# Mictronics/pluto-gps-sim

Measured on AMD Instinct MI355X. Metric: IQ samples/sec (whole node) at 16 channels; bit-exact int16 IQ vs CPU ref, higher is better.
Workload: dtype f64 NCOs (exact), i32 accumulate of packed int16 I/Q

## Files before the change

pluto-gps-sim_amd/csrc/gpsbb.hip:

```cpp
#include <hip/hip_runtime.h>

#include <algorithm>
#include <cctype>
#include <cmath>
#include <cstdio>
#include <cstdlib>
#include <cstring>
#include <new>
#include <condition_variable>
#include <functional>
#include <mutex>
#include <thread>
#include <chrono>
#include <vector>

#include "gpsbb.h"
#include "gpsbb_kernels.hip.h"
#include "gpsbb_noise.hip.h"
#include "gpsbb_interf.hip.h"
#include "gpsbb_level.hip.h"
#include "gpsbb_events.hip.h"
#include "gpsbb_dense.hip.h"
#include "gpsbb_despread.hip.h"
#include "gpsbb_despread_lags.hip.h"
// ... 3941 lines not shown
    HIPCHK(h, hipGetLastError());
    HIPCHK(h, hipStreamSynchronize(h->s_compute));
    HIPCHK(h, hipMemcpy(maxima, d_mx, mx_bytes, hipMemcpyDeviceToHost));
    HIPCHK(h, hipMemcpy(counts, d_cnt, cnt_bytes, hipMemcpyDeviceToHost));
    (void)hipFree(d_mx);
    (void)hipFree(d_cnt);
    if (which)
        *which = pl.ev_all_dense ? 2 : 1;
    return GPSBB_OK;
}

extern "C" int gpsbb_test_state_log2(gpsbb_batch_t *b)
{
    return b ? b->plan.st_log2 : GPSBB_E_BADARG;
}

static unsigned long long fnv1a(const void *p, size_t n)
{
    unsigned long long h = 0xcbf29ce484222325ull;
    for (size_t i = 0; i < n; i++)
        h = (h ^ ((const uint8_t *)p)[i]) * 0x100000001b3ull;
    return h;
}

template <class T>
static unsigned long long fnv1a(const std::vector<T> &v, bool defined = true)
{
    return defined ? fnv1a(v.data(), v.size() * sizeof(T)) : 0ull;
}

// ... 33 lines not shown
extern "C" int gpsbb_test_table_digest(gpsbb_batch_t *b, unsigned long long out[3])
{
    if (!b || !out || !b->ran || !b->plan.ev)
        return GPSBB_E_STATE;
    gpsbb *h = b->h;
    const BatchPlan &pl = b->plan;
    const int rc = gpsbb_sync(h);
    if (rc != GPSBB_OK)
        return rc;
    const BatchDev p = batch_dev(b, b->sets[b->last_set]);
    auto mix = [](unsigned long long z) { z ^= z >> 31; z *= 0xBF58476D1CE4E5B9ull; z ^= z >> 29; return z; };
    const size_t nst = (size_t)pl.nstates;
    const size_t nx = (size_t)pl.nblocks * 2 * pl.nch * nst, nn = (size_t)pl.nblocks * pl.nch * nst, ne = (size_t)pl.nblocks * pl.nch;
    const int dg = pl.ev_dense || (pl.flags & GPSBB_FIXED_CARRIER) ? 0 : (int)GPSBB_KNOB_LONG("GPSBB_EV_STATE_LOG2", GPSBB_EV_STATE_LOG2);
    const int tstep = 1 << (dg > pl.st_log2 ? dg : pl.st_log2);
    std::vector<unsigned long long> hx(nx);
    std::vector<uint32_t> hn(nn);
    std::vector<gpsbb_chan_state_t> he(ne);
    HIPCHK(h, hipMemcpy(hx.data(), p.tile_x, nx * 8, hipMemcpyDeviceToHost));
    HIPCHK(h, hipMemcpy(hn.data(), p.tile_nav, nn * 4, hipMemcpyDeviceToHost));
    HIPCHK(h, hipMemcpy(he.data(), p.end, ne * sizeof(gpsbb_chan_state_t), hipMemcpyDeviceToHost));
    out[0] = out[1] = out[2] = 0;
    std::vector<gpsbb_chan_t> hc(ne);
    HIPCHK(h, hipMemcpy(hc.data(), p.ch, ne * sizeof(gpsbb_chan_t), hipMemcpyDeviceToHost));
    for (size_t k = 0; k < ne; k++) {
        if (hc[k].prn <= 0)
            continue;
        const size_t blk = k / (size_t)pl.nch, i = k % (size_t)pl.nch;
        for (int kind = 0; kind < 2; kind++)
            for (int t = 0; t < pl.ntiles; t += tstep) {
                const size_t at = (blk * 2 * pl.nch + 2 * i + kind) * (size_t)pl.ntiles + t;
                out[0] += mix(hx[(blk * 2 * pl.nch + 2 * i + kind) * nst + (t >> pl.st_log2)] + 0x9E3779B97F4A7C15ull * (at + 1));
            }
        for (int t = 0; t < pl.ntiles; t += tstep) {
            const size_t at = k * (size_t)pl.ntiles + t;
            out[1] += mix((unsigned long long)(hn[k * nst + (t >> pl.st_log2)] & 3u) + 0x9E3779B97F4A7C15ull * (at + 1));
        }
        unsigned long long w[5];
        memcpy(w, &he[k], sizeof w);
        for (int q = 0; q < 4; q++)
            out[2] += mix(w[q] + 0x9E3779B97F4A7C15ull * (k * 5 + q + 1));
        out[2] += mix((unsigned long long)(uint32_t)he[k].codeCA + 0x9E3779B97F4A7C15ull * (k * 5 + 5));
    }
    return GPSBB_OK;
}

extern "C" void gpsbb_test_budgets(double out[3])
// ... 79 lines not shown
```

pluto-gps-sim_amd/csrc/gpsbb_despread.hip.h:

```cpp
#ifndef GPSBB_DESPREAD_HIP_H
#define GPSBB_DESPREAD_HIP_H

#include "gpsbb_dense.hip.h"
#include "gpsbb_noise.hip.h"
#include "gpsbb_interf.hip.h"

namespace gpsbb_impl {

constexpr int DS_WG = 256;
constexpr int DS_WAVES = DS_WG / 64;
constexpr int DS_CHUNK = 4;
constexpr int DS_SC16 = 0;

struct DsArgs {
    const uint32_t *iq;
    unsigned long long *out;
    unsigned long long *n_exact;
    int32_t *ctr;
    int seg_tiles, nseg, chunk, wgs_per_block;
    int shift8;
    uint32_t danger;
    NoiseArgs nz;
    const int2 *ntab;
    InterfArgs it;
};

typedef short ds_s16x2 __attribute__((ext_vector_type(2)));

struct DsLds {
    uint2 rep[2][512];
    uint32_t chips[GPSBB_MAX_CHAN][32];
};

__device__ __forceinline__ uint32_t ds_pair(int lo, int hi) { return ((uint32_t)lo & 0xffffu) | ((uint32_t)hi << 16); }

__device__ __noinline__ uint32_t ds_exact_sample(double xt, double yt, double S, double sc, uint32_t down, uint32_t nav, int n,
                                                 const uint32_t *chips)
{
    int64_t wraps = 0;
    const double x = code_jump(xt, sc, (int64_t)n, &wraps);
    const uint32_t neg = wraps > 0 ? (nav >> 1) & 1u : nav & 1u;
    const double cp = carr_jump(yt * (1.0 / 512.0), (down ? -S : S) * (1.0 / 512.0), (int64_t)n);
    const int it = (int)(cp * 512.0) & 511;
    const int ci = (int)x;
    const uint32_t bit = (chips[(ci >> 5) & 31] >> (ci & 31)) & 1u;
    return (uint32_t)it | (((bit ^ 1u) ^ neg) << 9);
}

__device__ __forceinline__ uint32_t ds_model_sample(double nn, double S, double sc, double yg, double xg, uint32_t flip, uint32_t nav,
                                                    const uint32_t *chips, uint32_t danger, bool &bad)
{
    const double y = __fma_rn(nn, S, yg), x = __fma_rn(nn, sc, xg);
    bad = min((uint32_t)__double2loint(y), (uint32_t)__double2loint(x)) < danger;
    const uint32_t it = ((uint32_t)__double2hiint(y) & 511u) ^ flip;
    uint32_t c = (uint32_t)__double2hiint(x) & 0xfffffu;
    const bool rolled = c >= (uint32_t)GPSBB_CA_LEN;
    c -= rolled ? (uint32_t)GPSBB_CA_LEN : 0u;
    const uint32_t bit = (chips[(c >> 5) & 31u] >> (c & 31u)) & 1u;
    const uint32_t neg = rolled ? (nav >> 1) & 1u : nav & 1u;
    return it | (((bit ^ 1u) ^ neg) << 9);
}

struct DsRepTab {
    const uint2 *rep;
    __device__ __forceinline__ void operator()(uint32_t idx, int *c, int *s) const
    {
        const uint32_t v = rep[idx].x;
// ... 98 lines not shown
            const int seg = wt / a.seg_tiles;
            if (seg != run_seg) {
                flush();
                run_seg = seg;
            }
            const int left = p.nsamp - wt * TILE - lane;
            uint32_t u[SPT];
#pragma unroll
            for (int j = 0; j < SPT; j++)
                u[j] = j * 64 < left ? iqb[(size_t)wt * TILE + j * 64 + lane] : 0u;
#pragma unroll
            for (int j = 0; j < SPT; j++)
                u[j] = j * 64 < left ? ds_view<VIEW, NOISE, INTERF>(u[j], (unsigned long long)b * (unsigned long long)p.nsamp +
                                                                              (unsigned long long)(wt * TILE + j * 64 + lane), a, ntab, L.rep[0])
                                     : 0u;
            const int g = wt >> SG;
            const double n0 = (double)((wt & ((1 << SG) - 1)) * TILE + lane);
            for (uint32_t mk = act_mask; mk; mk &= mk - 1) {
                const int i = __builtin_ctz(mk);
                const double S = scalar_load(&kb[i].S), sc = scalar_load(&kb[i].sc);
                const uint32_t down = scalar_load(&kb[i].down) != 0 ? 1u : 0u;
                const double xt = txb[(size_t)(2 * i) * nst + g], yt = txb[(size_t)(2 * i + 1) * nst + g];
                const uint32_t nav = tnb[(size_t)i * nst + g];
                const double yg = (down ? 512.0 - yt : yt) + guard, xg = xt + guard;
                const uint32_t flip = down ? 511u : 0u;
                const uint32_t *chips = L.chips[i];
                int pi = 0, pq = 0;
                uint32_t bad = 0u;
#pragma unroll
                for (int j = 0; j < SPT; j++) {
                    bool bj;
                    const uint32_t r = ds_model_sample(n0 + (double)(j * 64), S, sc, yg, xg, flip, nav, chips, a.danger, bj);
                    bad |= bj ? 1u << j : 0u;
                    const uint2 t = (&L.rep[0][0])[r];
                    pi = __builtin_amdgcn_sdot2(__builtin_bit_cast(ds_s16x2, u[j]), __builtin_bit_cast(ds_s16x2, t.x), pi, false);
                    pq = __builtin_amdgcn_sdot2(__builtin_bit_cast(ds_s16x2, u[j]), __builtin_bit_cast(ds_s16x2, t.y), pq, false);
                }
                if (__builtin_expect(__builtin_amdgcn_ballot_w64(bad != 0u) != 0ull, 0)) {
#pragma unroll 1
                    for (int j = 0; j < SPT; j++) {
                        if (!((bad >> j) & 1u) || j * 64 >= left)
                            continue;
                        uint32_t uw = 0u;
#pragma unroll
                        for (int q = 0; q < SPT; q++)
                            uw = q == j ? u[q] : uw;
                        bool bj;
                        const uint32_t rm = ds_model_sample(n0 + (double)(j * 64), S, sc, yg, xg, flip, nav, chips, a.danger, bj);
                        const uint32_t re = ds_exact_sample(xt, yt, S, sc, down, nav, (wt & ((1 << SG) - 1)) * TILE + j * 64 + lane, chips);
                        const uint2 tm = (&L.rep[0][0])[rm], te = (&L.rep[0][0])[re];
                        const ds_s16x2 uj = __builtin_bit_cast(ds_s16x2, uw);
                        pi += __builtin_amdgcn_sdot2(uj, __builtin_bit_cast(ds_s16x2, te.x), 0, false) -
                              __builtin_amdgcn_sdot2(uj, __builtin_bit_cast(ds_s16x2, tm.x), 0, false);
                        pq += __builtin_amdgcn_sdot2(uj, __builtin_bit_cast(ds_s16x2, te.y), 0, false) -
                              __builtin_amdgcn_sdot2(uj, __builtin_bit_cast(ds_s16x2, tm.y), 0, false);
                        n_exact++;
                    }
                }
                long long si = pi, sq = pq;
#pragma unroll
                for (int off = 32; off > 0; off >>= 1) {
                    si += __shfl_xor(si, off);
                    sq += __shfl_xor(sq, off);
                }
// ... 18 lines not shown
```

pluto-gps-sim_amd/csrc/gpsbb_despread_lags.hip.h:

```cpp
#ifndef GPSBB_DESPREAD_LAGS_HIP_H
#define GPSBB_DESPREAD_LAGS_HIP_H

#include "gpsbb_despread.hip.h"

namespace gpsbb_impl {

constexpr int DSL_MAX_LAGS = GPSBB_DESPREAD_MAX_LAGS;
constexpr int DSL_HALO = GPSBB_DESPREAD_MAX_LAG;
constexpr int DSL_STRIP = TILE + 2 * DSL_HALO;
constexpr int DSL_RED_ROW = 64 + 4;
static_assert(DSL_HALO == 64 && 2 * DSL_MAX_LAGS == 16 && GPSBB_MAX_CHAN == 16,
              "one halo group per side; lane (v, q) = (2 * lag + component, channel & 3), register set channel >> 2");

struct DslArgs {
    DsArgs d;
    int lags[DSL_MAX_LAGS];
    int nlags;
    int halo_lo, halo_hi;
};

template <int VIEW, bool NOISE, int SG, bool INTERF = false>
__global__ __launch_bounds__(DS_WG) void k_despread_lags(BatchDev p, DslArgs al)
{
    __shared__ DsLds L;
// ... 71 lines not shown
            __builtin_amdgcn_wave_barrier();
            const int m0 = wt * TILE - DSL_HALO + lane;
#pragma unroll 2
            for (int g = 0; g < SPT + 2; g++) {
                const int m = m0 + g * 64;
                const bool need = (g != 0 || al.halo_lo) && (g != SPT + 1 || al.halo_hi);
                uint32_t w = 0u;
                if (need && m >= 0 && m < p.nsamp)
                    w = ds_view<VIEW, NOISE, INTERF>(iqb[m], (unsigned long long)b * (unsigned long long)p.nsamp + (unsigned long long)m, a,
                                                     ntab, L.rep[0]);
                vw[g * 64 + lane] = w;
            }
            __builtin_amdgcn_fence(__ATOMIC_ACQ_REL, "workgroup");
            __builtin_amdgcn_wave_barrier();
            const int left = p.nsamp - wt * TILE - lane;
            const int g = wt >> SG;
            const int ns = (wt & ((1 << SG) - 1)) * TILE + lane;
            const double n0 = (double)ns;
            for (uint32_t mk = act_mask; mk; mk &= mk - 1) {
                const int i = __builtin_ctz(mk);
                const double S = scalar_load(&kb[i].S), sc = scalar_load(&kb[i].sc);
                const uint32_t down = scalar_load(&kb[i].down) != 0 ? 1u : 0u;
                const double xt = txb[(size_t)(2 * i) * nst + g], yt = txb[(size_t)(2 * i + 1) * nst + g];
                const uint32_t nav = tnb[(size_t)i * nst + g];
                const double yg = (down ? 512.0 - yt : yt) + guard, xg = xt + guard;
                const uint32_t flip = down ? 511u : 0u;
                const uint32_t *chips = L.chips[i];
                uint2 t[SPT];
                uint32_t bad = 0u;
#pragma unroll
                for (int j = 0; j < SPT; j++) {
                    bool bj;
                    const uint32_t r = ds_model_sample(n0 + (double)(j * 64), S, sc, yg, xg, flip, nav, chips, a.danger, bj);
                    const bool is = j * 64 < left;
                    bad |= bj && is ? 1u << j : 0u;
                    const uint2 tj = (&L.rep[0][0])[r];
                    t[j] = is ? tj : make_uint2(0u, 0u);
                }
                if (__builtin_expect(__builtin_amdgcn_ballot_w64(bad != 0u) != 0ull, 0)) {
#pragma unroll 1
                    for (int j = 0; j < SPT; j++) {
                        if (!((bad >> j) & 1u))
                            continue;
                        const uint32_t re = ds_exact_sample(xt, yt, S, sc, down, nav, ns + j * 64, chips);
                        const uint2 te = (&L.rep[0][0])[re];
#pragma unroll
                        for (int q = 0; q < SPT; q++)
                            t[q] = q == j ? te : t[q];
                        n_exact++;
                    }
                }
                __builtin_amdgcn_fence(__ATOMIC_ACQ_REL, "workgroup");
                __builtin_amdgcn_wave_barrier();
#pragma unroll 1
                for (int l = 0; l < nlags; l++) {
                    const int lag = __builtin_amdgcn_readfirstlane(lagv[l]);
                    const uint32_t *__restrict__ wl = vw + (DSL_HALO + lane + lag);
                    uint32_t w[SPT];
#pragma unroll
// ... 43 lines not shown
```

pluto-gps-sim_amd/csrc/gpsbb_events.hip.h:

```cpp
#ifndef GPSBB_EVENTS_HIP_H
#define GPSBB_EVENTS_HIP_H

#include <cstddef>
#include <type_traits>

#include "gpsbb_kernels.hip.h"

namespace gpsbb_impl {

#ifndef GPSBB_EV_WG
#define GPSBB_EV_WG 1024
#endif
constexpr int EV_WG = GPSBB_EV_WG;
constexpr int EV_WAVES = EV_WG / 64;
constexpr int EV_KC_MAX = 4;
constexpr int EV_AMP_PAD = EV_KC_MAX;
constexpr int EV_AMP_STRIDE = 512 + EV_AMP_PAD + 4;
constexpr int EV_CHIP_LEN = 1024 + 544;
constexpr int EV_KC_DENSE = EV_KC_MAX + 1;
#ifndef GPSBB_EV_CHUNK
#define GPSBB_EV_CHUNK 4
#endif
constexpr int EV_CHUNK = GPSBB_EV_CHUNK;
constexpr int PD_CHUNK = 2;
// ... 4 lines not shown
#define GPSBB_EV_MODEL_ERR_OWN 1
#endif
#ifndef EV_T_EPS
#define EV_T_EPS 0x1p-29
#endif
#define EV_GUARD 0x1p+20

#ifndef GPSBB_EV_STATE_LOG2
#define GPSBB_EV_STATE_LOG2 1
#endif
constexpr int EV_STATE_LOG2_MAX = 2;
static_assert(GPSBB_EV_STATE_LOG2 >= 0 && GPSBB_EV_STATE_LOG2 <= EV_STATE_LOG2_MAX, "state granule: 1, 2 or 4 tiles");
constexpr bool ev_granule_fits(int g) { return ((double)(TILE << g) + (double)(SPT - 1)) * 0x1p-44 + 1.5 * 0x1p-32 <= EV_MODEL_ERR; }
#ifdef GPSBB_EV_MODEL_ERR_OWN
static_assert(ev_granule_fits(EV_STATE_LOG2_MAX), "the model of the largest state granule must stay inside the error budget");
#endif

#define GPSBB_EV_SETTLE_CLAIM() asm volatile("s_waitcnt vmcnt(0)" ::: "memory")

constexpr int EV_CHIP_LEN_SHORT = 1104;
constexpr int EV_AMP_STRIDE_LONG = 512 + 272 + EV_AMP_PAD;
template <int AMP_STRIDE, int CHIP_LEN>
struct EvLdsT {
    static constexpr int AMP = AMP_STRIDE, CHIPS = CHIP_LEN;
    static constexpr bool UNMASKED = AMP_STRIDE >= EV_AMP_STRIDE_LONG;
    uint32_t amp[GPSBB_MAX_CHAN][AMP_STRIDE];
    uint32_t D[EV_WAVES][16][64];
    double tstate[EV_WAVES][2][2 * GPSBB_MAX_CHAN];
    double tstep[2 * GPSBB_MAX_CHAN];
    uint16_t chip2[GPSBB_MAX_CHAN][CHIP_LEN];
// ... 32 lines not shown
                 "ds_add_u32 %0, %3 offset:%4"
                 : "+v"(drow)
                 : "s"(wave << 4), "v"(pos_hi), "v"(v), "n"(offsetof(LDS, D))
                 );
}

__device__ __forceinline__ uint32_t signed_by(uint32_t x, uint32_t m) { return (x ^ m) - m; }

template <class T>
__device__ __forceinline__ T scalar_load(const T *p)
{
    typedef const __attribute__((address_space(4))) T *cptr_t;
    return *(cptr_t)(uintptr_t)p;
}

template <bool FIXED, class LDS>
__device__ __forceinline__ uint32_t ev_exact_run_body(LDS &L, int wave, int lane, int i, const EvConst *kbi, const double *tile_x,
                                                      int ntiles, uint32_t nb, int n_off, uint32_t fx_phase, int32_t fx_step)
{
    constexpr bool fixed = FIXED;
    const bool down = kbi->down != 0;
    const double S = down ? -kbi->S : kbi->S, sc = kbi->sc;
    const double xt = tile_x[(size_t)(2 * i) * ntiles], yt = tile_x[(size_t)(2 * i + 1) * ntiles];
    int64_t wraps = 0;
    double x = code_jump(xt, sc, (int64_t)n_off, &wraps);
    uint32_t dbm = (wraps > 0 ? (nb >> 1) & 1u : nb & 1u) ? 0xffffffffu : 0u;
    const uint32_t dbm_next = ((nb >> 1) & 1u) ? 0xffffffffu : 0u;
    const double s = S * (1.0 / 512.0);
    double cp = carr_jump(yt * (1.0 / 512.0), s, (int64_t)n_off);
    uint32_t prev = 0, first = 0;
    uint32_t ph = fx_phase + (uint32_t)n_off * (uint32_t)fx_step;
#pragma unroll 1
    for (int j = 0; j < SPT; j++) {
        const int it = fixed ? (int)((ph >> 16) & 0x1ffu)
                             : ((int)(cp * 512.0) & 511);
        const int ci = (int)x;
        const uint32_t m = (uint32_t)(int32_t)(int8_t)(L.chip2[i][ci] & 0xffu) ^ dbm;
        const uint32_t v = signed_by(L.amp[i][down ? 511 - it : it], m);
        if (j == 0)
            first = v;
        else
            __hip_atomic_fetch_add(&L.D[wave][j - 1][lane], v - prev, __ATOMIC_RELAXED, __HIP_MEMORY_SCOPE_WORKGROUP);
        prev = v;
        if (code_step(x, sc))
// ... 2 lines not shown
        ph += (uint32_t)fx_step;
    }
    return first;
}

struct EvFixed {
    const uint32_t *ph;
    const int32_t *st;
    int n0;
};

template <class LDS>
__device__ __noinline__ uint32_t ev_exact_run(LDS &L, int wave, int lane, int i, const EvConst *kbi, const double *tile_x,
                                              int ntiles, uint32_t nb, int n_off)
{
    return ev_exact_run_body<false>(L, wave, lane, i, kbi, tile_x, ntiles, nb, n_off, 0u, 0);
}
template <class LDS>
__device__ __noinline__ uint32_t ev_exact_run_fixed(LDS &L, int wave, int lane, int i, const EvConst *kbi, const double *tile_x,
                                                    int ntiles, uint32_t nb, int n_off, uint32_t fx_phase, int32_t fx_step)
{
    return ev_exact_run_body<true>(L, wave, lane, i, kbi, tile_x, ntiles, nb, n_off, fx_phase, fx_step);
}

struct EvK {
    double S, rS, sc, rsc;
    uint32_t danger;
    uint32_t chip_base;
    uint32_t amp_base;
};
constexpr uint32_t EV_GUARD_HI = 0x41300000u;
template <class LDS>
__device__ __forceinline__ EvK ev_load_k(const LDS &L, const EvConst *kb, int i)
{
    EvK k;
    typedef uint32_t u32x8 __attribute__((ext_vector_type(8)));
    typedef uint32_t u32x4 __attribute__((ext_vector_type(4)));
// ... 88 lines not shown
    EvExactAt a;
    if (!T.sg) {
        a.tile_x = T.tile_x;
        a.stride = T.ntiles;
        a.nb = ((T.dbits >> i) & 1u) | (((T.dnext >> i) & 1u) << 1);
        a.n_skip = 0;
    } else {
        const int nst = (T.ntiles + (1 << T.sg) - 1) >> T.sg, g = T.wt >> T.sg;
        a.tile_x = T.tile_x + g;
        a.stride = nst;
        a.nb = ((T.dbits >> i) & 1u) | (((T.dnext >> i) & 1u) << 1);
        a.n_skip = (T.wt & ((1 << T.sg) - 1)) * TILE;
    }
    return a;
}

template <int KC, bool DF, bool FIXED, class LDS>
__device__ __forceinline__ void ev_second(LDS &L, uint32_t &drow, int wave, int lane, int i, EvHalf<KC> &h, uint32_t db, uint32_t db_next,
                                          unsigned long long live_mask, const EvConst *kb, const EvTile &T,
                                          double off, uint32_t &acc0, unsigned long long *n_exact, const EvFixed &fx)
{
    const uint32_t ma = (uint32_t)(int32_t)(int8_t)(h.ch2 & 0xffu), mb = (uint32_t)(int32_t)(int8_t)(h.ch2 >> 8);
    uint32_t m0, m1;
    if (DF) {
        m0 = ma ^ (h.c0 >= 1023 ? db_next : db);
        m1 = mb ^ (h.c0 >= 1022 ? db_next : db);
    } else {
        m0 = ma ^ db;
        m1 = mb ^ db;
    }
    uint32_t hc = m0 == m1 ? EV_SAT_HI : h.hc;

    if (__builtin_expect(h.um != 0ull, 0)) {
        const unsigned long long um = h.um & live_mask;
        GPSBB_EV_SETTLE_CLAIM();
        if ((um >> lane) & 1ull) {
#pragma unroll
            for (int k = 0; k < KC; k++)
                h.hk[k] = EV_SAT_HI;
            hc = EV_SAT_HI;
            h.A[0] = 0;
            const EvExactAt x = ev_exact_at(T, i);
            if (FIXED)
                acc0 += ev_exact_run_fixed(L, wave, lane, i, kb + i, x.tile_x, x.stride, x.nb, x.n_skip + (int)off,
                                           fx.ph[i] + (uint32_t)fx.n0 * (uint32_t)fx.st[i], fx.st[i]);
            else
                acc0 += ev_exact_run(L, wave, lane, i, kb + i, x.tile_x, x.stride, x.nb, x.n_skip + (int)off);
            atomicAdd(n_exact, 1ull);
        }
    }

    {
        const uint32_t c = acc0 - m0;
        asm("v_xad_u32 %0, %1, %2, %3" : "=v"(acc0) : "v"(h.A[0]), "v"(m0), "v"(c));
    }
    uint32_t Ax = h.A[KC];
#pragma unroll
    for (int k = KC - 1; k >= 0; k--) {
        const bool before = h.hk[k] < hc;
        const uint32_t mk = before ? m0 : m1;
// ... 229 lines not shown
    const int ntw = p.ntiles;
    const int nch2 = 2 * p.nch;
    uint32_t mk[EV_KC_MAX];
    uint32_t mkd;
    {
        const bool act = lane < p.nch && cb[lane < p.nch ? lane : 0].prn > 0;
        const int kc = act ? kb[lane].kc : 0;
#pragma unroll
        for (int k = 0; k < EV_KC_MAX; k++)
            mk[k] = (uint32_t)__ballot(act && (kc == k + 1 || (k == 0 && kc < 1)));
        mkd = DENSE ? (uint32_t)__ballot(act && kc == EV_KC_DENSE) : 0u;
    }
    const bool chain_lane = lane < nch2;
    const bool mirror = chain_lane && (lane & 1) && kb[lane >> 1].down != 0;
    constexpr int sg = SG;
    const int nst = SG ? p.nstates : ntw;
    const double *__restrict__ txb = p.tile_x + (size_t)b * nst * nch2;
    const uint32_t *__restrict__ tnb = p.tile_nav + (size_t)b * p.nch * nst;
    const double off = (double)(lane * SPT);
    const double guard_w = EV_GUARD + ((chain_lane && !(FIXED && (lane & 1))) ? kb[lane >> 1].W : 0.0);
    const double mirror_at = FIXED ? 512.0 - 0x1p-16 : 512.0;
    unsigned long long *n_exact = p.hazards + 2;
    const uint32_t dwave = lds_addr_of(&L.D[wave][0][0]);
    const uint32_t d_col = dwave + (uint32_t)lane * 4u;
    const uint32_t t_wr = (dwave + (uint32_t)lane * 64u) ^ ((((uint32_t)lane >> 1) & 3u) << 4);
    const uint32_t t_rd = dwave + ((uint32_t)lane >> 2) * 64u + ((((uint32_t)lane & 3u) ^ (((uint32_t)lane >> 3) & 3u)) << 4);
    const uint32_t t_zero = dwave + (uint32_t)lane * 16u;
    uint32_t drow = (uint32_t)lane * 4u;

    int base = 0;
// ... 1 lines not shown
        base = atomicAdd(&p.tile_ctr[b], p.ev_chunk);
    base = __builtin_amdgcn_readfirstlane(base);
    int pos = 0;
    int pending = 0;
    unsigned tiles_rendered = 0;
    double ts_v = 0.0;
    uint32_t nav_v = 0;
    const auto stage_tile = [&](int t, uint32_t &dbits, uint32_t &dnext) {
        const int r = t & ((1 << sg) - 1);
        bool rolled_over = false;
        uint32_t ln = (uint32_t)lane;
        asm volatile("" : "+v"(ln));
        if (chain_lane) {
            double v = (mirror ? mirror_at - ts_v : ts_v) + guard_w;
            if (sg) {
                if (r)
                    v = __fma_rn(SG == 1 ? (double)TILE : (double)(r * TILE), L.tstep[ln], v);
                const uint32_t ip = (uint32_t)__double2hiint(v) - EV_GUARD_HI;
                const uint32_t red = (ln & 1u) ? (ip & ~511u) : (ip >= (uint32_t)GPSBB_CA_LEN + 1u ? (uint32_t)GPSBB_CA_LEN : 0u);
                v -= (double)red;
                rolled_over = !(ln & 1u) && red != 0u;
            }
            L.tstate[wave][0][ln] = v;
        }
        dbits = (uint32_t)__ballot(nav_v & 1u);
        dnext = (uint32_t)__ballot(nav_v & 2u);
        if (sg && r) {
            uint32_t ro = (uint32_t)__ballot(rolled_over) & 0x55555555u;
            ro = (ro | (ro >> 1)) & 0x33333333u;
            ro = (ro | (ro >> 2)) & 0x0f0f0f0fu;
            ro = (ro | (ro >> 4)) & 0x00ff00ffu;
            ro = (ro | (ro >> 8)) & 0x0000ffffu;
            dbits = (dbits & ~ro) | (dnext & ro);
        }
    };
    uint32_t t_dbits = 0u, t_dnext = 0u;
    const auto fetch_granule = [&](int g) {
        uint32_t ln = (uint32_t)lane;
        asm volatile("" : "+v"(ln));
        const uint32_t at = ln * (uint32_t)nst + (uint32_t)g;
        if (chain_lane)
            ts_v = txb[at];
        if (lane < p.nch)
            nav_v = tnb[at];
    };
    if (base < ntw) {
        fetch_granule(base >> sg);
        stage_tile(base, t_dbits, t_dnext);
    }
    while (base < ntw) {
        const int wt = base + pos;
        const int r = wt & ((1 << sg) - 1);
        EvTile T;
        T.ts = L.tstate[wave][0];
        T.tile_x = sg ? txb : txb + wt;
        T.ntiles = ntw;
        T.wt = wt;
// ... 153 lines not shown
```

pluto-gps-sim_amd/csrc/gpsbb_laps.hip.h:

```cpp
#ifndef GPSBB_LAPS_HIP_H
#define GPSBB_LAPS_HIP_H

#include "gpsbb_walk.hip.h"

namespace gpsbb_impl {

#ifdef GPSBB_LAP_WAVES
#define GPSBB_LAP_OCC __attribute__((amdgpu_waves_per_eu(GPSBB_LAP_WAVES, GPSBB_LAP_WAVES)))
#else
#define GPSBB_LAP_OCC
#endif
constexpr int LAP_WG = 256;
constexpr uint32_t LAPF_ACTIVE = 1u;
constexpr uint32_t LAPF_HEAD = 2u;
constexpr uint32_t LAPF_CONT = 4u;
constexpr uint32_t LAPF_CONST = 8u;
constexpr uint32_t LAPF_BAD = 16u;
constexpr uint32_t ST_LAP_PLAN = 8u;

struct LapBC {
    double phi;
    double s;
    double R1;
    double Rphi;
// ... 310 lines not shown
template <int KIND>
__device__ __forceinline__ void lap_enter_block(const BatchDev &p, const LapDev &L, int i, LapLane<KIND> &w)
{
    const LapBC bc = L.bc[((size_t)KIND * p.nch + i) * (size_t)p.nblocks + w.b];
    w.s = bc.s;
    w.bcflags = bc.flags;
    w.c0 = bc.c0;
    const uint64_t sb = f64_bits(bc.s);
    w.es = (int)((sb >> 52) & 0x7ff);
    w.tiemask = (sb << 1) == 0ull ? 0ull : walk_tiemask(sb);
    w.neg = bc.s < 0.0;
    w.tt = ((w.tiemask >> (((KIND == NCO_CARR ? 1022 : 1023 + 9) - w.es) & 63)) & 1ull) != 0ull;
    w.nmax = (w.b == w.bt) ? w.nt : p.nsamp;
}

template <int KIND, int SG = -1>
__device__ __forceinline__ void lap_nav_out(const BatchDev &p, int i, LapLane<KIND> &w, bool on, int n_excl, uint32_t bits)
{
    const uint32_t tsl = (uint32_t)__builtin_ctz(TILE) + (uint32_t)(SG >= 0 ? SG : p.st_log2);
    const int TS = 1 << tsl;
    typedef uint32_t lap_u4 __attribute__((ext_vector_type(4)));
    const int t = w.navt;
    int t_end = (int)(((uint32_t)n_excl + (uint32_t)(TS - 1)) >> tsl);
    t_end = t_end < p.nstates ? t_end : p.nstates;
    int cnt = on && t_end > t ? t_end - t : 0;
    if (cnt > 0)
        w.navt = t_end;
    if (!__ballot(cnt > 0))
        return;
    uint32_t *pn = p.tile_nav + ((size_t)w.b * (size_t)p.nch + i) * (size_t)p.nstates + t;
// ... 8 lines not shown
            }
        }
        if (quad)
            *reinterpret_cast<lap_u4 *>(pn) = b4;
        if (cnt > 0 && !oct && !quad)
            *pn = bits;
        const int adv = oct ? 8 : (quad ? 4 : (cnt > 0 ? 1 : 0));
        pn += adv;
        cnt -= adv;
    }
}

template <int KIND, bool WIDE, int SG = -1>
__device__ __forceinline__ void lap_emit_row(const BatchDev &p, int i, bool on, int b, int n, int k, double x, double S, uint32_t bits)
{
    const uint32_t tsl = (uint32_t)__builtin_ctz(TILE) + (uint32_t)(SG >= 0 ? SG : p.st_log2);
    const int TS = 1 << tsl;
    int t = (int)(((uint32_t)n + (uint32_t)(TS - 1)) >> tsl);
    int t_end = (int)((uint32_t)(n + k) >> tsl) + 1;
    t_end = t_end < p.nstates ? t_end : p.nstates;
    int cnt = on ? t_end - t : 0;
    cnt = cnt < 0 ? 0 : cnt;
    if (!__ballot(cnt > 0))
        return;
    double *__restrict__ tx = p.tile_x + ((size_t)b * (2 * (size_t)p.nch) + 2 * i + KIND) * (size_t)p.nstates;
    unsigned long long big = __ballot(cnt > 24);
    if (big && __popcll(big) <= 6) {
        const int lane = (int)__lane_id();
        while (big) {
            const int src = __builtin_ctzll(big);
            big &= big - 1;
            const int t0 = __builtin_amdgcn_readlane(t, src), c = __builtin_amdgcn_readlane(cnt, src);
            const int nn = __builtin_amdgcn_readlane(n, src);
            const double xx = bits_f64(readlane_u64(f64_bits(x), src)), SS = bits_f64(readlane_u64(f64_bits(S), src));
            const uint32_t bb = (uint32_t)__builtin_amdgcn_readlane((int)bits, src);
// ... 55 lines not shown
            }
        }
        if (one)
            *px = KIND == NCO_CARR ? mul_rn(v, 512.0) : v;
        const int adv = quad ? 4 : (pair ? 2 : (one ? 1 : 0));
        v = add_rn(quad || pair ? v3 : v, dv);
        px += adv;
        cnt -= adv;
    }
}

constexpr int LAP_BURST = 16;
template <int KIND, bool SNEG, bool EMIT, bool TIES, bool WIDE, int SG = -1>
__device__ __forceinline__ void lap_run(const BatchDev &p, int i, LapLane<KIND> &w, const bool was, const int L_burst)
{
    const uint32_t tsl = (uint32_t)__builtin_ctz(TILE) + (uint32_t)(SG >= 0 ? SG : p.st_log2);
    const int TS = 1 << tsl;
    constexpr int TOPEX = LapK<KIND>::TOPEX;
    constexpr int TOP = KIND == NCO_CARR ? 1022 : 1023 + 9;
    const double s = w.s;
    const int es = w.es, nmax = w.nmax;
    const bool any_tie = __ballot(was && w.tiemask != 0ull) != 0ull;
    const bool any_tt = TIES && __ballot(was && w.tt) != 0ull;
    const bool burst_ok = L_burst != 0 && !__ballot(was && es > TOP - 8);
    double x = w.x;
    int n = w.n;
    bool go = was, last_wrapped = false;
    const bool any_still = KIND == NCO_CARR && !SNEG && __ballot(was && s == 0.0) != 0ull;
    while (__ballot(go)) {
        if (any_still) {
            const bool still = go && s == 0.0 && x < 1.0;
            if (__ballot(still)) {
                const int k = still && nmax > n ? nmax - n : 0;
                if (EMIT && p.tile_x) {
                    const int t0 = (int)(((uint32_t)n + (uint32_t)(TS - 1)) >> tsl);
                    if (__ballot(still && (t0 << tsl) <= n + k && t0 < p.nstates))
                        lap_emit_row<KIND, WIDE, SG>(p, i, still, w.b, n, k, x, 0.0, w.bits);
                }
                if (still) {
                    n += k;
                    last_wrapped = k > 0 ? false : last_wrapped;
                    go = false;
                }
                continue;
            }
        }
#ifdef GPSBB_LAP_DEBUG
        if (__lane_id() == (unsigned)__builtin_ctzll(__ballot(go)))
            atomicAdd(p.hazards + 3, 1ull);
#endif
        const uint32_t hi = (uint32_t)__double2hiint(x);
// ... 57 lines not shown
        rs = __fma_rn(__fma_rn(-Sa, rs, 1.0), rs, rs);
        const double kq = fmin(room * rs, 2147483000.0);
        int ki = (int)kq;
        const double rem = __fma_rn(-(double)ki, Sa, room);
        ki += (rem < 0.0 ? -1 : 0) + (rem >= Sa ? 1 : 0);
        const int kcap = nmax - n;
        const int k = (expl || !(room >= Sa)) ? 0 : (ki < kcap ? ki : kcap);
        const double x1 = __fma_rn((double)k, S, x);
        if (KIND == NCO_CARR && __ballot(go && weird)) {
            if (go && ex >= TOPEX && !(hi >> 31))
                w.hz++;
        }
        const int n1 = n + k;
        if (EMIT && p.tile_x) {
            const int t0 = (int)(((uint32_t)n + (uint32_t)(TS - 1)) >> tsl);
            if (__ballot(go && (t0 << tsl) <= n1 && t0 < p.nstates))
                lap_emit_row<KIND, WIDE, SG>(p, i, go, w.b, n, k, x, S, w.bits);
        }
        const bool step = go && n1 < nmax;
        double x2 = add_rn(x1, s);
        bool wrapped;
        double xw;
        if (KIND == NCO_CARR) {
            wrapped = SNEG ? x2 < 0.0 : x2 >= 1.0;
            xw = add_rn(x2, SNEG ? 1.0 : -1.0);
        } else {
            wrapped = x2 >= 1023.0;
            xw = add_rn(x2, -1023.0);
        }
        wrapped = wrapped && step;
        if ((TIES || KIND == NCO_CODE) && __ballot(wrapped)) {
// ... 966 lines not shown
```

pluto-gps-sim_amd/csrc/gpsbb_modelerr.hip.h:

```cpp
#ifndef GPSBB_MODELERR_HIP_H
#define GPSBB_MODELERR_HIP_H

#include "gpsbb_dense.hip.h"

namespace gpsbb_impl {

enum {
    ME_Y0 = 0,
    ME_Y0_W,
    ME_TK,
    ME_TK_W,
    ME_X0,
    ME_X0_W,
    ME_TC,
    ME_TC_W,
    ME_PURE_Y,
    ME_PURE_X,
    ME_W_UNITS,
    ME_NQ
};
static_assert(ME_NQ == 11, "GPSBB_TEST_ME_NQ");
enum { MEC_BAD = 0, MEC_DANGER, MEC_LANES, MEC_ALWAYS, MEC_NQ };

__device__ __forceinline__ void me_max(double *slot, double v)
// ... 162 lines not shown
    else if (bad)
        A.bad++;
}

__global__ __launch_bounds__(256) void k_model_err_ev(BatchDev p, double *mx, unsigned long long *cnt)
{
    const size_t gid = (size_t)blockIdx.x * blockDim.x + threadIdx.x;
    const int wt = (int)(gid % (size_t)p.ntiles);
    const int i = (int)((gid / (size_t)p.ntiles) % (size_t)p.nch);
    const size_t b = gid / ((size_t)p.ntiles * p.nch);
    if (b >= (size_t)p.nblocks)
        return;
    if (p.ch[b * p.nch + i].prn <= 0)
        return;
    const EvConst kb = p.evc[b * p.nch + i];
    const int sg = p.st_log2, nst = p.nstates, r = wt & ((1 << sg) - 1);
    const double *txb = p.tile_x + b * (size_t)nst * 2 * p.nch;
    const double ts_x_g = txb[(size_t)(2 * i) * nst + (wt >> sg)], ts_y = txb[(size_t)(2 * i + 1) * nst + (wt >> sg)];
    const bool down = kb.down != 0;
    const bool fixed = p.kph0 != nullptr;
    const double guard_w = EV_GUARD + kb.W;
    const double ts_y_g = down ? (fixed ? 512.0 - 0x1p-16 : 512.0) - ts_y : ts_y;
    double ytg = ts_y_g + (fixed ? EV_GUARD : guard_w), xtg = ts_x_g + guard_w;
    int red_laps = 0, red_wraps = 0;
    double ts_y_m = ts_y_g, ts_x = ts_x_g;
    if (sg) {
        ytg = __fma_rn((double)(r * TILE), kb.S, ytg);
        xtg = __fma_rn((double)(r * TILE), kb.sc, xtg);
        const uint32_t iy = (uint32_t)__double2hiint(ytg) - EV_GUARD_HI, ix = (uint32_t)__double2hiint(xtg) - EV_GUARD_HI;
        const uint32_t ry = iy & ~511u, rx = ix >= (uint32_t)GPSBB_CA_LEN + 1u ? (uint32_t)GPSBB_CA_LEN : 0u;
        ytg -= (double)ry;
        xtg -= (double)rx;
        red_laps = (int)(ry >> 9);
        red_wraps = rx ? 1 : 0;
    }
    MeTruth T;
    T.cp = fixed ? 0.0 : ts_y * (1.0 / 512.0);
    T.s = fixed ? 0.0 : (down ? -kb.S : kb.S) * (1.0 / 512.0);
    T.x = ts_x_g;
    T.sc = kb.sc;
    T.laps = T.wraps = 0;
    T.down = down;
    T.fixed = fixed;
    T.st = fixed ? (uint32_t)p.kstep[b * p.nch + i] : 0u;
    T.ph = fixed ? p.kph0[b * p.nch + i] + (uint32_t)(wt - r) * (uint32_t)TILE * T.st : 0u;
    for (int n = 0; n < r * TILE; n++)
        T.step();
    T.laps -= red_laps;
    T.wraps -= red_wraps;
    if (sg) {
        ts_y_m = T.u();
        ts_x = T.ux();
    }
    MeAcc A;
    for (int q = 0; q < ME_NQ; q++)
        A.mx[q] = 0.0;
    A.bad = A.danger = A.lanes = A.always = 0;
    A.up(ME_W_UNITS, kb.W * 0x1p+32);
    for (int lane = 0; lane < 64; lane++) {
        const int n0 = wt * TILE + lane * SPT;
// ... 117 lines not shown
```

pluto-gps-sim_amd/csrc/gpsbb_testhooks.h:

```cpp
#ifndef GPSBB_TESTHOOKS_H
#define GPSBB_TESTHOOKS_H
#include <stdint.h>
#ifdef __cplusplus
extern "C" {
#endif

typedef struct gpsbb_test_row {
    int32_t n0;
    uint32_t nav;
    uint64_t xb;
    int64_t inc;
} gpsbb_test_row_t;

double gpsbb_test_carr_jump(double x, double s, long long n);
double gpsbb_test_code_jump(double x, double s, long long n, long long *wraps);
int gpsbb_test_build_rows(int kind, double x0, double s, unsigned nav0, int nsamp, gpsbb_test_row_t *rows,
                          int cap, double *x_end, unsigned *nav_end);
int gpsbb_test_build_rows_f64(int kind, double x0, double s, unsigned nav0, int nsamp, gpsbb_test_row_t *rows,
                              int cap, double *x_end, unsigned *nav_end);
unsigned long long gpsbb_test_row_bound(int kind, double s_abs, int nsamp);
double gpsbb_test_carr_predict(double x0, double s, int n);
double gpsbb_test_fixed_tile_index(unsigned ph0, int step, int t);

#define GPSBB_TEST_PLAN_NQ 38
struct gpsbb_chan;
int gpsbb_test_plan(const struct gpsbb_chan *ch, int nblocks, int nch, double delt, int nsamp, unsigned flags, const int opt[5],
                    int carry, const int *carry_prn, double *carry_phase, const int *fixed_prev_prn,
                    const uint32_t *fixed_prev_phase, unsigned long long out[GPSBB_TEST_PLAN_NQ]);

#define GPSBB_TEST_ME_NQ 11
#define GPSBB_TEST_MEC_NQ 4
struct gpsbb_batch;
int gpsbb_test_model_err(struct gpsbb_batch *b, double *maxima, unsigned long long *counts, int *which);
unsigned long long gpsbb_test_despread_exact(struct gpsbb_batch *b);
float gpsbb_test_despread_ms(struct gpsbb_batch *b);
void gpsbb_test_budgets(double out[3]);

#ifdef __cplusplus
}
#endif
#endif
```

Measured before the change: 617.6 billion.

## Store carrier NCO tile states at a coarser granule than code states

```diff
diff --git a/pluto-gps-sim_amd/csrc/gpsbb.hip b/pluto-gps-sim_amd/csrc/gpsbb.hip
--- a/pluto-gps-sim_amd/csrc/gpsbb.hip
+++ b/pluto-gps-sim_amd/csrc/gpsbb.hip
@@ -3979,6 +3979,10 @@
 {
     return b ? b->plan.st_log2 : GPSBB_E_BADARG;
 }
+extern "C" int gpsbb_test_state_log2_carr(gpsbb_batch_t *b)
+{
+    return b ? ev_carr_log2(b->plan.st_log2) : GPSBB_E_BADARG;
+}
 
 static unsigned long long fnv1a(const void *p, size_t n)
 {
@@ -4042,6 +4046,7 @@
     const size_t nx = (size_t)pl.nblocks * 2 * pl.nch * nst, nn = (size_t)pl.nblocks * pl.nch * nst, ne = (size_t)pl.nblocks * pl.nch;
     const int dg = pl.ev_dense || (pl.flags & GPSBB_FIXED_CARRIER) ? 0 : (int)GPSBB_KNOB_LONG("GPSBB_EV_STATE_LOG2", GPSBB_EV_STATE_LOG2);
     const int tstep = 1 << (dg > pl.st_log2 ? dg : pl.st_log2);
+    const int gc = ev_carr_log2(pl.st_log2), tstep_carr = 1 << ev_carr_log2(dg > pl.st_log2 ? dg : pl.st_log2);
     std::vector<unsigned long long> hx(nx);
     std::vector<uint32_t> hn(nn);
     std::vector<gpsbb_chan_state_t> he(ne);
@@ -4056,9 +4061,10 @@
             continue;
         const size_t blk = k / (size_t)pl.nch, i = k % (size_t)pl.nch;
         for (int kind = 0; kind < 2; kind++)
-            for (int t = 0; t < pl.ntiles; t += tstep) {
+            for (int t = 0; t < pl.ntiles; t += kind == NCO_CARR ? tstep_carr : tstep) {
                 const size_t at = (blk * 2 * pl.nch + 2 * i + kind) * (size_t)pl.ntiles + t;
-                out[0] += mix(hx[(blk * 2 * pl.nch + 2 * i + kind) * nst + (t >> pl.st_log2)] + 0x9E3779B97F4A7C15ull * (at + 1));
+                out[0] += mix(hx[(blk * 2 * pl.nch + 2 * i + kind) * nst + (t >> (kind == NCO_CARR ? gc : pl.st_log2))] +
+                              0x9E3779B97F4A7C15ull * (at + 1));
             }
         for (int t = 0; t < pl.ntiles; t += tstep) {
             const size_t at = k * (size_t)pl.ntiles + t;
diff --git a/pluto-gps-sim_amd/csrc/gpsbb_despread.hip.h b/pluto-gps-sim_amd/csrc/gpsbb_despread.hip.h
--- a/pluto-gps-sim_amd/csrc/gpsbb_despread.hip.h
+++ b/pluto-gps-sim_amd/csrc/gpsbb_despread.hip.h
@@ -34,23 +34,33 @@
 
 __device__ __forceinline__ uint32_t ds_pair(int lo, int hi) { return ((uint32_t)lo & 0xffffu) | ((uint32_t)hi << 16); }
 
-__device__ __noinline__ uint32_t ds_exact_sample(double xt, double yt, double S, double sc, uint32_t down, uint32_t nav, int n,
-                                                 const uint32_t *chips)
+__device__ __forceinline__ uint32_t ds_exact_sample_body(double xt, double yt, double S, double sc, uint32_t down, uint32_t nav, int n,
+                                                         int ny, const uint32_t *chips)
 {
     int64_t wraps = 0;
     const double x = code_jump(xt, sc, (int64_t)n, &wraps);
     const uint32_t neg = wraps > 0 ? (nav >> 1) & 1u : nav & 1u;
-    const double cp = carr_jump(yt * (1.0 / 512.0), (down ? -S : S) * (1.0 / 512.0), (int64_t)n);
+    const double cp = carr_jump(yt * (1.0 / 512.0), (down ? -S : S) * (1.0 / 512.0), (int64_t)ny);
     const int it = (int)(cp * 512.0) & 511;
     const int ci = (int)x;
     const uint32_t bit = (chips[(ci >> 5) & 31] >> (ci & 31)) & 1u;
     return (uint32_t)it | (((bit ^ 1u) ^ neg) << 9);
 }
-
-__device__ __forceinline__ uint32_t ds_model_sample(double nn, double S, double sc, double yg, double xg, uint32_t flip, uint32_t nav,
+__device__ __noinline__ uint32_t ds_exact_sample(double xt, double yt, double S, double sc, uint32_t down, uint32_t nav, int n,
+                                                 const uint32_t *chips)
+{
+    return ds_exact_sample_body(xt, yt, S, sc, down, nav, n, n, chips);
+}
+__device__ __noinline__ uint32_t ds_exact_sample_2g(double xt, double yt, double S, double sc, uint32_t down, uint32_t nav, int n, int ny,
+                                                    const uint32_t *chips)
+{
+    return ds_exact_sample_body(xt, yt, S, sc, down, nav, n, ny, chips);
+}
+
+__device__ __forceinline__ uint32_t ds_model_sample(double nn, double nny, double S, double sc, double yg, double xg, uint32_t flip, uint32_t nav,
                                                     const uint32_t *chips, uint32_t danger, bool &bad)
 {
-    const double y = __fma_rn(nn, S, yg), x = __fma_rn(nn, sc, xg);
+    const double y = __fma_rn(nny, S, yg), x = __fma_rn(nn, sc, xg);
     bad = min((uint32_t)__double2loint(y), (uint32_t)__double2loint(x)) < danger;
     const uint32_t it = ((uint32_t)__double2hiint(y) & 511u) ^ flip;
     uint32_t c = (uint32_t)__double2hiint(x) & 0xfffffu;
@@ -179,13 +189,15 @@
                 u[j] = j * 64 < left ? ds_view<VIEW, NOISE, INTERF>(u[j], (unsigned long long)b * (unsigned long long)p.nsamp +
                                                                               (unsigned long long)(wt * TILE + j * 64 + lane), a, ntab, L.rep[0])
                                      : 0u;
-            const int g = wt >> SG;
-            const double n0 = (double)((wt & ((1 << SG) - 1)) * TILE + lane);
+            constexpr int GC = ev_carr_log2(SG);
+            const int g = wt >> SG, gy = wt >> GC;
+            const int ns = (wt & ((1 << SG) - 1)) * TILE + lane, nsy = GC == SG ? ns : (wt & ((1 << GC) - 1)) * TILE + lane;
+            const double n0 = (double)ns, n0y = (double)nsy;
             for (uint32_t mk = act_mask; mk; mk &= mk - 1) {
                 const int i = __builtin_ctz(mk);
                 const double S = scalar_load(&kb[i].S), sc = scalar_load(&kb[i].sc);
                 const uint32_t down = scalar_load(&kb[i].down) != 0 ? 1u : 0u;
-                const double xt = txb[(size_t)(2 * i) * nst + g], yt = txb[(size_t)(2 * i + 1) * nst + g];
+                const double xt = txb[(size_t)(2 * i) * nst + g], yt = txb[(size_t)(2 * i + 1) * nst + gy];
                 const uint32_t nav = tnb[(size_t)i * nst + g];
                 const double yg = (down ? 512.0 - yt : yt) + guard, xg = xt + guard;
                 const uint32_t flip = down ? 511u : 0u;
@@ -195,7 +207,7 @@
 #pragma unroll
                 for (int j = 0; j < SPT; j++) {
                     bool bj;
-                    const uint32_t r = ds_model_sample(n0 + (double)(j * 64), S, sc, yg, xg, flip, nav, chips, a.danger, bj);
+                    const uint32_t r = ds_model_sample(n0 + (double)(j * 64), n0y + (double)(j * 64), S, sc, yg, xg, flip, nav, chips, a.danger, bj);
                     bad |= bj ? 1u << j : 0u;
                     const uint2 t = (&L.rep[0][0])[r];
                     pi = __builtin_amdgcn_sdot2(__builtin_bit_cast(ds_s16x2, u[j]), __builtin_bit_cast(ds_s16x2, t.x), pi, false);
@@ -211,8 +223,9 @@
                         for (int q = 0; q < SPT; q++)
                             uw = q == j ? u[q] : uw;
                         bool bj;
-                        const uint32_t rm = ds_model_sample(n0 + (double)(j * 64), S, sc, yg, xg, flip, nav, chips, a.danger, bj);
-                        const uint32_t re = ds_exact_sample(xt, yt, S, sc, down, nav, (wt & ((1 << SG) - 1)) * TILE + j * 64 + lane, chips);
+                        const uint32_t rm = ds_model_sample(n0 + (double)(j * 64), n0y + (double)(j * 64), S, sc, yg, xg, flip, nav, chips, a.danger, bj);
+                        const uint32_t re = GC == SG ? ds_exact_sample(xt, yt, S, sc, down, nav, ns + j * 64, chips)
+                                                     : ds_exact_sample_2g(xt, yt, S, sc, down, nav, ns + j * 64, nsy + j * 64, chips);
                         const uint2 tm = (&L.rep[0][0])[rm], te = (&L.rep[0][0])[re];
                         const ds_s16x2 uj = __builtin_bit_cast(ds_s16x2, uw);
                         pi += __builtin_amdgcn_sdot2(uj, __builtin_bit_cast(ds_s16x2, te.x), 0, false) -
diff --git a/pluto-gps-sim_amd/csrc/gpsbb_despread_lags.hip.h b/pluto-gps-sim_amd/csrc/gpsbb_despread_lags.hip.h
--- a/pluto-gps-sim_amd/csrc/gpsbb_despread_lags.hip.h
+++ b/pluto-gps-sim_amd/csrc/gpsbb_despread_lags.hip.h
@@ -109,14 +109,15 @@
             __builtin_amdgcn_fence(__ATOMIC_ACQ_REL, "workgroup");
             __builtin_amdgcn_wave_barrier();
             const int left = p.nsamp - wt * TILE - lane;
-            const int g = wt >> SG;
-            const int ns = (wt & ((1 << SG) - 1)) * TILE + lane;
-            const double n0 = (double)ns;
+            constexpr int GC = ev_carr_log2(SG);
+            const int g = wt >> SG, gy = wt >> GC;
+            const int ns = (wt & ((1 << SG) - 1)) * TILE + lane, nsy = GC == SG ? ns : (wt & ((1 << GC) - 1)) * TILE + lane;
+            const double n0 = (double)ns, n0y = (double)nsy;
             for (uint32_t mk = act_mask; mk; mk &= mk - 1) {
                 const int i = __builtin_ctz(mk);
                 const double S = scalar_load(&kb[i].S), sc = scalar_load(&kb[i].sc);
                 const uint32_t down = scalar_load(&kb[i].down) != 0 ? 1u : 0u;
-                const double xt = txb[(size_t)(2 * i) * nst + g], yt = txb[(size_t)(2 * i + 1) * nst + g];
+                const double xt = txb[(size_t)(2 * i) * nst + g], yt = txb[(size_t)(2 * i + 1) * nst + gy];
                 const uint32_t nav = tnb[(size_t)i * nst + g];
                 const double yg = (down ? 512.0 - yt : yt) + guard, xg = xt + guard;
                 const uint32_t flip = down ? 511u : 0u;
@@ -126,7 +127,7 @@
 #pragma unroll
                 for (int j = 0; j < SPT; j++) {
                     bool bj;
-                    const uint32_t r = ds_model_sample(n0 + (double)(j * 64), S, sc, yg, xg, flip, nav, chips, a.danger, bj);
+                    const uint32_t r = ds_model_sample(n0 + (double)(j * 64), n0y + (double)(j * 64), S, sc, yg, xg, flip, nav, chips, a.danger, bj);
                     const bool is = j * 64 < left;
                     bad |= bj && is ? 1u << j : 0u;
                     const uint2 tj = (&L.rep[0][0])[r];
@@ -137,7 +138,8 @@
                     for (int j = 0; j < SPT; j++) {
                         if (!((bad >> j) & 1u))
                             continue;
-                        const uint32_t re = ds_exact_sample(xt, yt, S, sc, down, nav, ns + j * 64, chips);
+                        const uint32_t re = GC == SG ? ds_exact_sample(xt, yt, S, sc, down, nav, ns + j * 64, chips)
+                                                     : ds_exact_sample_2g(xt, yt, S, sc, down, nav, ns + j * 64, nsy + j * 64, chips);
                         const uint2 te = (&L.rep[0][0])[re];
 #pragma unroll
                         for (int q = 0; q < SPT; q++)
diff --git a/pluto-gps-sim_amd/csrc/gpsbb_events.hip.h b/pluto-gps-sim_amd/csrc/gpsbb_events.hip.h
--- a/pluto-gps-sim_amd/csrc/gpsbb_events.hip.h
+++ b/pluto-gps-sim_amd/csrc/gpsbb_events.hip.h
@@ -42,6 +42,18 @@
 constexpr bool ev_granule_fits(int g) { return ((double)(TILE << g) + (double)(SPT - 1)) * 0x1p-44 + 1.5 * 0x1p-32 <= EV_MODEL_ERR; }
 #ifdef GPSBB_EV_MODEL_ERR_OWN
 static_assert(ev_granule_fits(EV_STATE_LOG2_MAX), "the model of the largest state granule must stay inside the error budget");
+#endif
+constexpr bool ev_carr_granule_fits(int gc) { return ((double)(TILE << gc) + (double)(SPT - 1)) * 0x1p-45 + 1.5 * 0x1p-32 <= EV_MODEL_ERR; }
+constexpr int ev_carr_log2(int g)
+{
+    int gc = g >= 1 ? (g + 1 < EV_STATE_LOG2_MAX ? g + 1 : EV_STATE_LOG2_MAX) : 0;
+    while (gc > g && !ev_carr_granule_fits(gc))
+        gc--;
+    return gc;
+}
+#ifdef GPSBB_EV_MODEL_ERR_OWN
+static_assert(ev_carr_granule_fits(EV_STATE_LOG2_MAX), "the carrier model of the largest state granule must stay inside the error budget");
+static_assert(EV_STATE_LOG2_MAX == 2, "ev_second names the one granule whose carrier's differs (ev_exact_run_2g<1>)");
 #endif
 
 #define GPSBB_EV_SETTLE_CLAIM() asm volatile("s_waitcnt vmcnt(0)" ::: "memory")
@@ -104,20 +116,21 @@
     return *(cptr_t)(uintptr_t)p;
 }
 
-template <bool FIXED, class LDS>
+template <bool FIXED, bool TWO_G = false, class LDS>
 __device__ __forceinline__ uint32_t ev_exact_run_body(LDS &L, int wave, int lane, int i, const EvConst *kbi, const double *tile_x,
-                                                      int ntiles, uint32_t nb, int n_off, uint32_t fx_phase, int32_t fx_step)
+                                                      int ntiles, uint32_t nb, int n_off, const double *tile_y, int n_off_y,
+                                                      uint32_t fx_phase, int32_t fx_step)
 {
     constexpr bool fixed = FIXED;
     const bool down = kbi->down != 0;
     const double S = down ? -kbi->S : kbi->S, sc = kbi->sc;
-    const double xt = tile_x[(size_t)(2 * i) * ntiles], yt = tile_x[(size_t)(2 * i + 1) * ntiles];
+    const double xt = tile_x[(size_t)(2 * i) * ntiles], yt = (TWO_G ? tile_y : tile_x)[(size_t)(2 * i + 1) * ntiles];
     int64_t wraps = 0;
     double x = code_jump(xt, sc, (int64_t)n_off, &wraps);
     uint32_t dbm = (wraps > 0 ? (nb >> 1) & 1u : nb & 1u) ? 0xffffffffu : 0u;
     const uint32_t dbm_next = ((nb >> 1) & 1u) ? 0xffffffffu : 0u;
     const double s = S * (1.0 / 512.0);
-    double cp = carr_jump(yt * (1.0 / 512.0), s, (int64_t)n_off);
+    double cp = carr_jump(yt * (1.0 / 512.0), s, (int64_t)(TWO_G ? n_off_y : n_off));
     uint32_t prev = 0, first = 0;
     uint32_t ph = fx_phase + (uint32_t)n_off * (uint32_t)fx_step;
 #pragma unroll 1
@@ -150,13 +163,22 @@
 __device__ __noinline__ uint32_t ev_exact_run(LDS &L, int wave, int lane, int i, const EvConst *kbi, const double *tile_x,
                                               int ntiles, uint32_t nb, int n_off)
 {
-    return ev_exact_run_body<false>(L, wave, lane, i, kbi, tile_x, ntiles, nb, n_off, 0u, 0);
+    return ev_exact_run_body<false>(L, wave, lane, i, kbi, tile_x, ntiles, nb, n_off, nullptr, 0, 0u, 0);
+}
+template <int SG, class LDS>
+__device__ __noinline__ uint32_t ev_exact_run_2g(LDS &L, int wave, int lane, int i, const EvConst *kbi, const double *tile_x, int nst,
+                                                 uint32_t wt_nb, int off)
+{
+    constexpr int GC = ev_carr_log2(SG);
+    const int wt = (int)(wt_nb >> 2);
+    return ev_exact_run_body<false, true>(L, wave, lane, i, kbi, tile_x + (wt >> SG), nst, wt_nb & 3u, (wt & ((1 << SG) - 1)) * TILE + off,
+                                          tile_x + (wt >> GC), (wt & ((1 << GC) - 1)) * TILE + off, 0u, 0);
 }
 template <class LDS>
 __device__ __noinline__ uint32_t ev_exact_run_fixed(LDS &L, int wave, int lane, int i, const EvConst *kbi, const double *tile_x,
                                                     int ntiles, uint32_t nb, int n_off, uint32_t fx_phase, int32_t fx_step)
 {
-    return ev_exact_run_body<true>(L, wave, lane, i, kbi, tile_x, ntiles, nb, n_off, fx_phase, fx_step);
+    return ev_exact_run_body<true>(L, wave, lane, i, kbi, tile_x, ntiles, nb, n_off, nullptr, 0, fx_phase, fx_step);
 }
 
 struct EvK {
@@ -275,6 +297,7 @@
     }
     return a;
 }
+__device__ __forceinline__ bool ev_exact_2g(const EvTile &T) { return ev_carr_log2(T.sg) != T.sg; }
 
 template <int KC, bool DF, bool FIXED, class LDS>
 __device__ __forceinline__ void ev_second(LDS &L, uint32_t &drow, int wave, int lane, int i, EvHalf<KC> &h, uint32_t db, uint32_t db_next,
@@ -305,6 +328,9 @@
             if (FIXED)
                 acc0 += ev_exact_run_fixed(L, wave, lane, i, kb + i, x.tile_x, x.stride, x.nb, x.n_skip + (int)off,
                                            fx.ph[i] + (uint32_t)fx.n0 * (uint32_t)fx.st[i], fx.st[i]);
+            else if (ev_exact_2g(T))
+                acc0 += ev_exact_run_2g<1>(L, wave, lane, i, kb + i, T.tile_x, (T.ntiles + 1) >> 1,
+                                           ((uint32_t)T.wt << 2) | ((T.dbits >> i) & 1u) | (((T.dnext >> i) & 1u) << 1), (int)off);
             else
                 acc0 += ev_exact_run(L, wave, lane, i, kb + i, x.tile_x, x.stride, x.nb, x.n_skip + (int)off);
             atomicAdd(n_exact, 1ull);
@@ -564,6 +590,7 @@
     const bool chain_lane = lane < nch2;
     const bool mirror = chain_lane && (lane & 1) && kb[lane >> 1].down != 0;
     constexpr int sg = SG;
+    constexpr int gc = ev_carr_log2(SG);
     const int nst = SG ? p.nstates : ntw;
     const double *__restrict__ txb = p.tile_x + (size_t)b * nst * nch2;
     const uint32_t *__restrict__ tnb = p.tile_nav + (size_t)b * p.nch * nst;
@@ -595,8 +622,13 @@
         if (chain_lane) {
             double v = (mirror ? mirror_at - ts_v : ts_v) + guard_w;
             if (sg) {
-                if (r)
-                    v = __fma_rn(SG == 1 ? (double)TILE : (double)(r * TILE), L.tstep[ln], v);
+                if (gc == sg) {
+                    if (r)
+                        v = __fma_rn(SG == 1 ? (double)TILE : (double)(r * TILE), L.tstep[ln], v);
+                } else if (t & ((1 << gc) - 1)) {
+                    const uint32_t rk = (uint32_t)t & ((ln & 1u) ? (1u << gc) - 1u : (1u << sg) - 1u);
+                    v = __fma_rn((double)(rk * (uint32_t)TILE), L.tstep[ln], v);
+                }
                 const uint32_t ip = (uint32_t)__double2hiint(v) - EV_GUARD_HI;
                 const uint32_t red = (ln & 1u) ? (ip & ~511u) : (ip >= (uint32_t)GPSBB_CA_LEN + 1u ? (uint32_t)GPSBB_CA_LEN : 0u);
                 v -= (double)red;
@@ -621,7 +653,7 @@
         asm volatile("" : "+v"(ln));
         const uint32_t at = ln * (uint32_t)nst + (uint32_t)g;
         if (chain_lane)
-            ts_v = txb[at];
+            ts_v = txb[gc == sg ? at : at - ((ln & 1u) ? (uint32_t)g - ((uint32_t)g >> (gc - sg)) : 0u)];
         if (lane < p.nch)
             nav_v = tnb[at];
     };
diff --git a/pluto-gps-sim_amd/csrc/gpsbb_laps.hip.h b/pluto-gps-sim_amd/csrc/gpsbb_laps.hip.h
--- a/pluto-gps-sim_amd/csrc/gpsbb_laps.hip.h
+++ b/pluto-gps-sim_amd/csrc/gpsbb_laps.hip.h
@@ -2,6 +2,7 @@
 #define GPSBB_LAPS_HIP_H
 
 #include "gpsbb_walk.hip.h"
+#include "gpsbb_events.hip.h"
 
 namespace gpsbb_impl {
 
@@ -348,6 +349,20 @@
     w.nmax = (w.b == w.bt) ? w.nt : p.nsamp;
 }
 
+template <int KIND, int SG>
+__device__ __forceinline__ uint32_t lap_tsl(const BatchDev &p)
+{
+    const int g = SG >= 0 ? SG : p.st_log2;
+    return (uint32_t)__builtin_ctz(TILE) + (uint32_t)(KIND == NCO_CARR ? ev_carr_log2(g) : g);
+}
+template <int KIND, int SG>
+__device__ __forceinline__ int lap_nstates(const BatchDev &p)
+{
+    if (KIND != NCO_CARR || (SG >= 0 && ev_carr_log2(SG) == SG))
+        return p.nstates;
+    const int gc = ev_carr_log2(SG >= 0 ? SG : p.st_log2);
+    return (p.ntiles + (1 << gc) - 1) >> gc;
+}
 template <int KIND, int SG = -1>
 __device__ __forceinline__ void lap_nav_out(const BatchDev &p, int i, LapLane<KIND> &w, bool on, int n_excl, uint32_t bits)
 {
@@ -386,11 +401,12 @@
 template <int KIND, bool WIDE, int SG = -1>
 __device__ __forceinline__ void lap_emit_row(const BatchDev &p, int i, bool on, int b, int n, int k, double x, double S, uint32_t bits)
 {
-    const uint32_t tsl = (uint32_t)__builtin_ctz(TILE) + (uint32_t)(SG >= 0 ? SG : p.st_log2);
+    const uint32_t tsl = lap_tsl<KIND, SG>(p);
+    const int nstates = lap_nstates<KIND, SG>(p);
     const int TS = 1 << tsl;
     int t = (int)(((uint32_t)n + (uint32_t)(TS - 1)) >> tsl);
     int t_end = (int)((uint32_t)(n + k) >> tsl) + 1;
-    t_end = t_end < p.nstates ? t_end : p.nstates;
+    t_end = t_end < nstates ? t_end : nstates;
     int cnt = on ? t_end - t : 0;
     cnt = cnt < 0 ? 0 : cnt;
     if (!__ballot(cnt > 0))
@@ -476,7 +492,8 @@
 template <int KIND, bool SNEG, bool EMIT, bool TIES, bool WIDE, int SG = -1>
 __device__ __forceinline__ void lap_run(const BatchDev &p, int i, LapLane<KIND> &w, const bool was, const int L_burst)
 {
-    const uint32_t tsl = (uint32_t)__builtin_ctz(TILE) + (uint32_t)(SG >= 0 ? SG : p.st_log2);
+    const uint32_t tsl = lap_tsl<KIND, SG>(p);
+    const int nstates = lap_nstates<KIND, SG>(p);
     const int TS = 1 << tsl;
     constexpr int TOPEX = LapK<KIND>::TOPEX;
     constexpr int TOP = KIND == NCO_CARR ? 1022 : 1023 + 9;
@@ -496,7 +513,7 @@
                 const int k = still && nmax > n ? nmax - n : 0;
                 if (EMIT && p.tile_x) {
                     const int t0 = (int)(((uint32_t)n + (uint32_t)(TS - 1)) >> tsl);
-                    if (__ballot(still && (t0 << tsl) <= n + k && t0 < p.nstates))
+                    if (__ballot(still && (t0 << tsl) <= n + k && t0 < nstates))
                         lap_emit_row<KIND, WIDE, SG>(p, i, still, w.b, n, k, x, 0.0, w.bits);
                 }
                 if (still) {
@@ -584,7 +601,7 @@
         const int n1 = n + k;
         if (EMIT && p.tile_x) {
             const int t0 = (int)(((uint32_t)n + (uint32_t)(TS - 1)) >> tsl);
-            if (__ballot(go && (t0 << tsl) <= n1 && t0 < p.nstates))
+            if (__ballot(go && (t0 << tsl) <= n1 && t0 < nstates))
                 lap_emit_row<KIND, WIDE, SG>(p, i, go, w.b, n, k, x, S, w.bits);
         }
         const bool step = go && n1 < nmax;
diff --git a/pluto-gps-sim_amd/csrc/gpsbb_modelerr.hip.h b/pluto-gps-sim_amd/csrc/gpsbb_modelerr.hip.h
--- a/pluto-gps-sim_amd/csrc/gpsbb_modelerr.hip.h
+++ b/pluto-gps-sim_amd/csrc/gpsbb_modelerr.hip.h
@@ -200,9 +200,9 @@
     if (p.ch[b * p.nch + i].prn <= 0)
         return;
     const EvConst kb = p.evc[b * p.nch + i];
-    const int sg = p.st_log2, nst = p.nstates, r = wt & ((1 << sg) - 1);
+    const int sg = p.st_log2, gc = ev_carr_log2(sg), nst = p.nstates, r = wt & ((1 << sg) - 1), ry_t = wt & ((1 << gc) - 1);
     const double *txb = p.tile_x + b * (size_t)nst * 2 * p.nch;
-    const double ts_x_g = txb[(size_t)(2 * i) * nst + (wt >> sg)], ts_y = txb[(size_t)(2 * i + 1) * nst + (wt >> sg)];
+    const double ts_x_g = txb[(size_t)(2 * i) * nst + (wt >> sg)], ts_y = txb[(size_t)(2 * i + 1) * nst + (wt >> gc)];
     const bool down = kb.down != 0;
     const bool fixed = p.kph0 != nullptr;
     const double guard_w = EV_GUARD + kb.W;
@@ -211,7 +211,7 @@
     int red_laps = 0, red_wraps = 0;
     double ts_y_m = ts_y_g, ts_x = ts_x_g;
     if (sg) {
-        ytg = __fma_rn((double)(r * TILE), kb.S, ytg);
+        ytg = __fma_rn((double)(ry_t * TILE), kb.S, ytg);
         xtg = __fma_rn((double)(r * TILE), kb.sc, xtg);
         const uint32_t iy = (uint32_t)__double2hiint(ytg) - EV_GUARD_HI, ix = (uint32_t)__double2hiint(xtg) - EV_GUARD_HI;
         const uint32_t ry = iy & ~511u, rx = ix >= (uint32_t)GPSBB_CA_LEN + 1u ? (uint32_t)GPSBB_CA_LEN : 0u;
@@ -230,6 +230,11 @@
     T.fixed = fixed;
     T.st = fixed ? (uint32_t)p.kstep[b * p.nch + i] : 0u;
     T.ph = fixed ? p.kph0[b * p.nch + i] + (uint32_t)(wt - r) * (uint32_t)TILE * T.st : 0u;
+    T.sc = 0.0;
+    for (int n = 0; n < (ry_t - r) * TILE; n++)
+        T.step();
+    T.sc = kb.sc;
+    T.wraps = 0;
     for (int n = 0; n < r * TILE; n++)
         T.step();
     T.laps -= red_laps;
diff --git a/pluto-gps-sim_amd/csrc/gpsbb_testhooks.h b/pluto-gps-sim_amd/csrc/gpsbb_testhooks.h
--- a/pluto-gps-sim_amd/csrc/gpsbb_testhooks.h
+++ b/pluto-gps-sim_amd/csrc/gpsbb_testhooks.h
@@ -34,6 +34,8 @@
 int gpsbb_test_model_err(struct gpsbb_batch *b, double *maxima, unsigned long long *counts, int *which);
 unsigned long long gpsbb_test_despread_exact(struct gpsbb_batch *b);
 float gpsbb_test_despread_ms(struct gpsbb_batch *b);
+int gpsbb_test_state_log2(struct gpsbb_batch *b);
+int gpsbb_test_state_log2_carr(struct gpsbb_batch *b);
 void gpsbb_test_budgets(double out[3]);
 
 #ifdef __cplusplus
```

Result: faster. 626.8 billion, median of 6 (+1.5%).
